# headupinclouds/cvsteer

Hardware: AMD Instinct MI355X
Metric: Mpix/s for G2+H2 7-basis filter+steer at 4096x4096 f32; % HBM roofline (higher is better)
Workload: dtype f32

## Files before the change

cvsteer_amd/csrc/cvs_api.cpp:

```cpp
#include <hip/hip_runtime_api.h>

#include <algorithm>
#include <atomic>
#include <chrono>
#include <condition_variable>
#include <cmath>
#include <cstdio>
#include <cstdlib>
#include <cstring>
#include <limits>
#include <map>
#include <mutex>
#include <set>
#include <tuple>
#include <new>
#include <string>
#include <thread>
#include <vector>

#include "cvs_context.h"

using namespace cvs;

namespace {
// ... 191 lines not shown
    for (int o = 0; o < 5; ++o)
        if ((rc = out_ref(c, outs[o], a.out[o]))) return rc;
    PointOp op = h->kind == CVS_KIND_G2 ? (map ? OP_G2_STEER_MAP : OP_G2_STEER_SCALAR)
                                        : (map ? OP_G4_STEER_MAP : OP_G4_STEER_SCALAR);
    a.nt_stores = use_nt_stores(h, (size_t)a.rows * a.cols);
    a.nt_loads = a.nt_stores;
    HIP_TRY(h, launch_point(op, a, h->stream));
    return finish(c);
}

int g4_pipe_stage(cvs_handle h, const cvs_plane* const outs[8], int nframes, size_t out_fstride)
{
    Call c;
    int rc = begin(h, c, {outs[0], outs[1], outs[2], outs[3], outs[4], outs[5], outs[6], outs[7]});
    if (rc) return rc;
    G4PipeArgs a{};
    a.rows = h->rows;
    a.cols = h->cols;
    a.frames = nframes;
    a.atan_mode = h->atan_mode;
    a.find_on_e = h->find_on;
    for (int p = 0; p < h->nb; ++p) {
        const PlaneRef r = state_ref(h, p);
        a.in[p] = {r.p, r.pitch, h->frame_stride};
    }
    if (h->persist) {
        for (int i = 0; i < 5; ++i) {
            const PlaneRef r = state_ref(h, h->nb + i);
            a.out[G4P_C1 + i] = {r.p, r.pitch, h->frame_stride};
        }
    }
    for (int k = 0; k < 8; ++k) {
        PlaneRef r;
        if ((rc = out_ref(c, outs[k], r))) return rc;
        a.out[G4P_G + k] = {r.p, r.pitch, out_fstride};
    }
    a.nt_stores = use_nt_stores(h, (size_t)a.rows * a.cols * nframes);
    a.nt_loads = a.nt_stores;
    HIP_TRY(h, launch_g4_pipeline(a, h->stream));
    h->have_basis = h->have_orient = h->persist != 0;
    return finish(c);
}

int g4_pipeline_one(cvs_handle h, const cvs_plane* image, const cvs_plane* const outs[8], int nframes, int frame)
{
    const int rc = do_setup(h, image, CVS_SETUP_BASIS, false, 0.f, nullptr, nullptr, nullptr, nframes, frame);
    return rc ? rc : g4_pipe_stage(h, outs, 1, 0);
}

int g4_pipeline_frames(cvs_handle h, const cvs_plane* images, int n, const cvs_plane* outs, bool all_dev)
{
    auto frame_outs = [&](int i, const cvs_plane* po[8]) {
        for (int k = 0; k < 8; ++k) po[k] = (outs && outs[(size_t)i * 8 + k].data) ? &outs[(size_t)i * 8 + k] : nullptr;
    };
    bool block = all_dev;
    ptrdiff_t d_out = 0;
    bool have_stride = false;
    for (int i = 1; i < n && block; ++i)
        for (int k = 0; k < 8 && block && outs; ++k) {
            const cvs_plane &o0 = outs[k], &oi = outs[(size_t)i * 8 + k];
            if ((o0.data == nullptr) != (oi.data == nullptr)) block = false;
            else if (o0.data) {
                const ptrdiff_t dk = oi.data - o0.data;
                if (!have_stride) { d_out = dk / i; have_stride = true; }
                block = dk == d_out * i && d_out > 0 && oi.step == o0.step;
            }
        }
    int rc;
    if (!block) {
        for (int i = 0; i < n; ++i) {
            const cvs_plane* po[8];
            frame_outs(i, po);
            if ((rc = g4_pipeline_one(h, &images[i], po, n, i))) return rc;
        }
        h->cur_frame = 0;
        return CVS_OK;
    }
    for (int i = 0; i < n; ++i)
        if ((rc = do_setup(h, &images[i], CVS_SETUP_BASIS, false, 0.f, nullptr, nullptr, nullptr, n, i))) return rc;
    h->cur_frame = 0;
    const cvs_plane* po[8];
    frame_outs(0, po);
    return g4_pipe_stage(h, po, n, (size_t)d_out);
}

}

extern "C" {

int cvs_abi_version(void) { return CVS_ABI_VERSION; }

const char* cvs_status_string(int s)
{
    switch (s) {
        case CVS_OK: return "ok";
        case CVS_E_BADARG: return "bad argument";
        case CVS_E_SIZE: return "bad size";
        case CVS_E_HIP: return "HIP error";
        case CVS_E_NOMEM: return "out of memory";
        case CVS_E_STATE: return "state not available";
        case CVS_E_UNSUPPORTED: return "unsupported for this kind";
    }
    return "unknown status";
}

int cvs_num_basis(int kind) { return host_num_basis(kind); }

int cvs_make_taps(int kind, int idx, int width, float spacing, float* out)
{
    return host_make_taps(kind, idx, width, spacing, out) ? CVS_E_BADARG : CVS_OK;
}

int cvs_basis_taps(int kind, int p, int* kx, int* ky) { return host_basis_taps(kind, p, kx, ky) ? CVS_E_BADARG : CVS_OK; }

int cvs_steer_weights(int kind, float theta, float* out) { return host_steer_weights(kind, theta, out) ? CVS_E_BADARG : CVS_OK; }

int cvs_create(int kind, int width, float spacing, int device, cvs_handle* out)
{
    if (!out) return CVS_E_BADARG;
    *out = nullptr;
    const int nb = host_num_basis(kind);
    if (nb == 0 || width < 1 || width > kMaxWidth) return CVS_E_BADARG;
    int ndev = 0;
    if (hipGetDeviceCount(&ndev) != hipSuccess || ndev <= 0) return CVS_E_HIP;
    if (device < 0 || device >= ndev) return CVS_E_BADARG;
    if (hipSetDevice(device) != hipSuccess) return CVS_E_HIP;
    cvs_context* h = new (std::nothrow) cvs_context();
    if (!h) return CVS_E_NOMEM;
    h->kind = kind;
    h->width = width;
    h->spacing = spacing;
    h->nb = nb;
    h->device = device;
    std::memset(h->taps, 0, sizeof(h->taps));
    for (int i = 0; i < nb; ++i) host_make_taps(kind, i, width, spacing, h->taps[i]);
    const EnvOpts eo = env_opts();
    if (eo.autotune >= 0) h->autotune = eo.autotune;
    if (eo.layout >= 0) h->layout = eo.layout;
    if (eo.pyr_strip >= 0) h->pyr_strip = eo.pyr_strip;
    *out = h;
    return CVS_OK;
}

int cvs_destroy(cvs_handle h)
{
    if (!h) return CVS_E_BADARG;
    (void)hipSetDevice(h->device);
    release_state(h);
    if (h->arena || h->frame_tab || h->point_out) (void)hipStreamSynchronize(h->stream);
    if (h->arena) (void)hipFree(h->arena);
    if (h->frame_tab) (void)hipFree(h->frame_tab);
    if (h->point_out) (void)hipFree(h->point_out);
    if (h->ev_order) (void)hipEventDestroy(h->ev_order);
    for (hipEvent_t e : h->band_ev) (void)hipEventDestroy(e);
    if (h->s_up) (void)hipStreamDestroy(h->s_up);
    if (h->s_down) (void)hipStreamDestroy(h->s_down);
    delete h;
    return CVS_OK;
}

int cvs_release_cached_memory(void)
{
    pool_release_all();
    return CVS_OK;
}

const char* cvs_last_error(cvs_handle h) { return h ? h->err.c_str() : "null handle"; }

int cvs_set_stream(cvs_handle h, void* s)
{
    if (!h) return CVS_E_BADARG;
    hipStream_t ns = static_cast<hipStream_t>(s);
    if (ns == h->stream) return CVS_OK;
    hipStreamCaptureStatus c0 = hipStreamCaptureStatusNone, c1 = hipStreamCaptureStatusNone;
    (void)hipStreamIsCapturing(h->stream, &c0);
    (void)hipStreamIsCapturing(ns, &c1);
    (void)hipGetLastError();
    if (h->used && c0 == hipStreamCaptureStatusNone && c1 == hipStreamCaptureStatusNone) {
        HIP_TRY(h, hipSetDevice(h->device));
        if (!h->ev_order) HIP_TRY(h, hipEventCreateWithFlags(&h->ev_order, hipEventDisableTiming));
        HIP_TRY(h, hipEventRecord(h->ev_order, h->stream));
        HIP_TRY(h, hipStreamWaitEvent(ns, h->ev_order, 0));
    }
    h->stream = ns;
    return CVS_OK;
}

int cvs_set_option(cvs_handle h, int option, int value)
{
    if (!h) return CVS_E_BADARG;
    switch (option) {
        case CVS_OPT_ATAN_MODE:
            if (value != 0 && value != 1) return fail(h, CVS_E_BADARG, "atan mode");
            h->atan_mode = value;
            return CVS_OK;
        case CVS_OPT_STRIP_ROWS:
            if (value < 0 || value > 1 << 20) return fail(h, CVS_E_BADARG, "strip rows");
            h->strip_rows = value;
            return CVS_OK;
        case CVS_OPT_FIND_ON:
            if (value != 0 && value != 1) return fail(h, CVS_E_BADARG, "find_on");
            h->find_on = value;
            return CVS_OK;
        case CVS_OPT_G4_EXTENSIONS:
            if (value != 0 && value != 1) return fail(h, CVS_E_BADARG, "g4 extensions");
            h->g4_ext = value;
            return CVS_OK;
        case CVS_OPT_PERSIST_STATE:
            if (value != 0 && value != 1) return fail(h, CVS_E_BADARG, "persist");
            h->persist = value;
            return CVS_OK;
        case CVS_OPT_AUTOTUNE:
            if (value != 0 && value != 1) return fail(h, CVS_E_BADARG, "autotune");
            h->autotune = value;
            return CVS_OK;
        case CVS_OPT_BLOCK_ORDER:
            if (value != -1 && value != 0 && value != kOrderXcdColumns && value != kOrderDynamic) return fail(h, CVS_E_BADARG, "block order");
            h->block_order = value;
            return CVS_OK;
        case CVS_OPT_HOST_OVERLAP:
            if (value != 0 && value != 1) return fail(h, CVS_E_BADARG, "host overlap");
            h->host_overlap = value;
            return CVS_OK;
        case CVS_OPT_STATE_LAYOUT:
            if (value < 0 || value > 3) return fail(h, CVS_E_BADARG, "state layout");
            h->layout = value;
            return CVS_OK;
    }
    return fail(h, CVS_E_BADARG, "unknown option");
}

int cvs_get_option(cvs_handle h, int option, int* value)
{
    if (!h || !value) return CVS_E_BADARG;
    switch (option) {
        case CVS_OPT_ATAN_MODE: *value = h->atan_mode; return CVS_OK;
        case CVS_OPT_STRIP_ROWS: *value = h->strip_rows; return CVS_OK;
        case CVS_OPT_FIND_ON: *value = h->find_on; return CVS_OK;
        case CVS_OPT_BLOCK_ORDER: *value = h->block_order; return CVS_OK;
        case CVS_OPT_HOST_OVERLAP: *value = h->host_overlap; return CVS_OK;
        case CVS_OPT_AUTOTUNE: *value = h->autotune; return CVS_OK;
        case CVS_OPT_PERSIST_STATE: *value = h->persist; return CVS_OK;
        case CVS_OPT_G4_EXTENSIONS: *value = h->g4_ext; return CVS_OK;
        case CVS_OPT_STATE_LAYOUT: *value = h->layout; return CVS_OK;
    }
    return fail(h, CVS_E_BADARG, "unknown option");
}

int cvs_get_launch_info(cvs_handle h, cvs_launch_info* out)
{
    if (!h || !out) return CVS_E_BADARG;
    const uint32_t n = out->struct_size;
    if (n < sizeof(uint32_t)) return fail(h, CVS_E_BADARG, "cvs_launch_info.struct_size not set");
    cvs_launch_info li = h->last;
    li.struct_size = (uint32_t)std::min<size_t>(n, sizeof(li));
    std::memcpy(out, &li, li.struct_size);
    return CVS_OK;
}

int cvs_taps(cvs_handle h, int idx, float* out)
{
    if (!h || !out || idx < 0 || idx >= h->nb) return CVS_E_BADARG;
    std::memcpy(out, h->taps[idx], (2 * h->width + 1) * sizeof(float));
    return CVS_OK;
}

int cvs_kind(cvs_handle h, int* kind, int* width, float* spacing)
{
    if (!h) return CVS_E_BADARG;
    if (kind) *kind = h->kind;
    if (width) *width = h->width;
    if (spacing) *spacing = h->spacing;
    return CVS_OK;
}

int cvs_shape(cvs_handle h, int* rows, int* cols)
{
    if (!h) return CVS_E_BADARG;
    if (rows) *rows = h->have_basis ? h->rows : 0;
    if (cols) *cols = h->have_basis ? h->cols : 0;
    return CVS_OK;
}

int cvs_sync(cvs_handle h)
{
    if (!h) return CVS_E_BADARG;
    HIP_TRY(h, hipSetDevice(h->device));
    HIP_TRY(h, hipStreamSynchronize(h->stream));
    return CVS_OK;
}

int cvs_setup(cvs_handle h, const cvs_plane* image, unsigned flags)
{
    return do_setup(h, image, flags, false, 0.f, nullptr, nullptr);
}

int cvs_setup_steer(cvs_handle h, const cvs_plane* image, unsigned flags, float theta, const cvs_plane* g, const cvs_plane* hq)
{
    return do_setup(h, image, flags, true, theta, g, hq);
}

int cvs_setup_pyr(cvs_handle h, const cvs_plane* image, unsigned flags, const cvs_plane* next_level)
{
    if (!h) return CVS_E_BADARG;
    if (!next_level) return fail(h, CVS_E_BADARG, "next_level");
    return do_setup(h, image, flags, false, 0.f, nullptr, nullptr, nullptr, 1, 0, 0, 0, next_level);
// ... 520 lines not shown
```

cvsteer_amd/csrc/cvs_batch.cpp:

```cpp
#include <dlfcn.h>
#include <hip/hip_runtime_api.h>
#include <rccl/rccl.h>

#include <algorithm>
#include <cstdio>
#include <cstdlib>
#include <cstring>
#include <condition_variable>
#include <mutex>
#include <new>
#include <string>
#include <thread>
#include <vector>

#include "cvsteer_hip.h"

namespace {

struct Rccl {
    void* so = nullptr;
    ncclResult_t (*GetUniqueId)(ncclUniqueId*) = nullptr;
    ncclResult_t (*CommInitRank)(ncclComm_t*, int, ncclUniqueId, int) = nullptr;
    ncclResult_t (*CommInitAll)(ncclComm_t*, int, const int*) = nullptr;
    ncclResult_t (*CommDestroy)(ncclComm_t) = nullptr;
    ncclResult_t (*GroupStart)() = nullptr;
    ncclResult_t (*GroupEnd)() = nullptr;
    ncclResult_t (*Send)(const void*, size_t, ncclDataType_t, int, ncclComm_t, hipStream_t) = nullptr;
    ncclResult_t (*Recv)(void*, size_t, ncclDataType_t, int, ncclComm_t, hipStream_t) = nullptr;
    ncclResult_t (*Broadcast)(const void*, void*, size_t, ncclDataType_t, int, ncclComm_t, hipStream_t) = nullptr;
    ncclResult_t (*AllReduce)(const void*, void*, size_t, ncclDataType_t, ncclRedOp_t, ncclComm_t, hipStream_t) = nullptr;
    const char* (*GetErrorString)(ncclResult_t) = nullptr;
    std::string why;
};

Rccl* rccl(std::string* why = nullptr)
{
    static Rccl r;
    static std::once_flag once;
    std::call_once(once, [] {
        const char* env = std::getenv("CVS_RCCL_LIB");
        const char* names[] = {env, "librccl.so.1", "librccl.so", "/opt/rocm/lib/librccl.so.1", "/opt/rocm/lib/librccl.so"};
        for (const char* n : names) {
            if (!n || !*n) continue;
            r.so = dlopen(n, RTLD_NOW | RTLD_GLOBAL);
            if (r.so) break;
        }
        if (!r.so) {
            r.why = std::string("cannot load librccl: ") + (dlerror() ? dlerror() : "not found");
            return;
        }
        bool ok = true;
        auto sym = [&](const char* name) {
            void* p = dlsym(r.so, name);
            if (!p) { ok = false; r.why = std::string("librccl lacks ") + name; }
            return p;
        };
        r.GetUniqueId = reinterpret_cast<decltype(r.GetUniqueId)>(sym("ncclGetUniqueId"));
        r.CommInitRank = reinterpret_cast<decltype(r.CommInitRank)>(sym("ncclCommInitRank"));
        r.CommInitAll = reinterpret_cast<decltype(r.CommInitAll)>(sym("ncclCommInitAll"));
        r.CommDestroy = reinterpret_cast<decltype(r.CommDestroy)>(sym("ncclCommDestroy"));
        r.GroupStart = reinterpret_cast<decltype(r.GroupStart)>(sym("ncclGroupStart"));
        r.GroupEnd = reinterpret_cast<decltype(r.GroupEnd)>(sym("ncclGroupEnd"));
        r.Send = reinterpret_cast<decltype(r.Send)>(sym("ncclSend"));
        r.Recv = reinterpret_cast<decltype(r.Recv)>(sym("ncclRecv"));
        r.Broadcast = reinterpret_cast<decltype(r.Broadcast)>(sym("ncclBroadcast"));
        r.AllReduce = reinterpret_cast<decltype(r.AllReduce)>(sym("ncclAllReduce"));
        r.GetErrorString = reinterpret_cast<decltype(r.GetErrorString)>(sym("ncclGetErrorString"));
        if (!ok) {
            dlclose(r.so);
            r.so = nullptr;
        }
    });
    if (!r.so && why) *why = r.why;
    return r.so ? &r : nullptr;
}

void shard_range(int n, int world, int rank, int* lo, int* hi)
{
    *lo = (int)(((long long)rank * n + world - 1) / world);
    *hi = (int)(((long long)(rank + 1) * n + world - 1) / world);
}

enum { TRANSPORT_NONE = 0, TRANSPORT_RCCL = 1, TRANSPORT_COPY = 2 };

struct DevBuf {
    float* p = nullptr;
    size_t elems = 0;
};

struct Slot {
    int rank = 0, device = 0;
    hipStream_t stream = nullptr;
    cvs_handle h = nullptr;
    std::vector<cvs_handle> level;
    std::vector<DevBuf> level_img;
    ncclComm_t comm = nullptr;
    DevBuf in, out, image;
    DevBuf out8;
    int last_n = 0, last_k = 0, last_rows = 0, last_cols = 0;
    bool last_staged = false;
    hipEvent_t ev[4] = {nullptr, nullptr, nullptr, nullptr};
    hipStream_t up = nullptr, down = nullptr;
    std::vector<hipEvent_t> host_ev;
    int* agree = nullptr;
};

}

struct cvs_batch_context {
    int kind = 0, width = 0, world = 0, transport = TRANSPORT_NONE;
    int g4_ext = 0;
    float spacing = 0.f;
    float u8_gain = 0.f;
    std::vector<Slot> slots;
    int pyr_levels = 0, pyr_root = 0;
    std::string err;
};

namespace {

int fail(cvs_batch b, int code, const std::string& what)
{
    if (b) b->err = what;
    return code;
}

#define B_HIP(b, expr)                                                                                   \
    do {                                                                                                 \
        hipError_t e__ = (expr);                                                                         \
        if (e__ != hipSuccess) return fail(b, e__ == hipErrorOutOfMemory ? CVS_E_NOMEM : CVS_E_HIP,      \
                                           std::string(#expr) + ": " + hipGetErrorString(e__));         \
    } while (0)

#define B_NCCL(b, expr)                                                                                  \
    do {                                                                                                 \
        ncclResult_t r__ = (expr);                                                                       \
        if (r__ != ncclSuccess) return fail(b, CVS_E_HIP, std::string(#expr) + ": " + rccl()->GetErrorString(r__)); \
    } while (0)

#define B_CVS(b, h, expr)                                                                                \
    do {                                                                                                 \
        int rc__ = (expr);                                                                               \
        if (rc__ != CVS_OK) return fail(b, rc__, std::string(#expr) + ": " + cvs_last_error(h));         \
    } while (0)

int reserve(cvs_batch b, Slot& s, DevBuf& buf, size_t elems)
{
    if (elems <= buf.elems) return CVS_OK;
    B_HIP(b, hipSetDevice(s.device));
    if (buf.p) {
        B_HIP(b, hipStreamSynchronize(s.stream));
        B_HIP(b, hipFree(buf.p));
        buf = DevBuf();
    }
    B_HIP(b, hipMalloc(&buf.p, elems * sizeof(float)));
    buf.elems = elems;
    return CVS_OK;
}

Slot* local(cvs_batch b, int rank)
{
    for (Slot& s : b->slots)
        if (s.rank == rank) return &s;
    return nullptr;
}

int init_slot(cvs_batch b, Slot& s)
// ... 75 lines not shown
        return g.end(b);
    }
    for (const Move& m : moves) {
        Slot* s = local(b, m.src_rank);
        Slot* d = local(b, m.dst_rank);
        if (!s || !d) return fail(b, CVS_E_UNSUPPORTED, "copy transport needs both ranks in this process");
        B_HIP(b, hipSetDevice(s->device));
        hipEvent_t e;
        B_HIP(b, hipEventCreateWithFlags(&e, hipEventDisableTiming));
        B_HIP(b, hipEventRecord(e, s->stream));
        B_HIP(b, hipSetDevice(d->device));
        B_HIP(b, hipStreamWaitEvent(d->stream, e, 0));
        B_HIP(b, hipMemcpyAsync(m.dst, m.src, m.count * sizeof(float), hipMemcpyDeviceToDevice, d->stream));
        hipEvent_t done;
        B_HIP(b, hipEventCreateWithFlags(&done, hipEventDisableTiming));
        B_HIP(b, hipEventRecord(done, d->stream));
        B_HIP(b, hipSetDevice(s->device));
        B_HIP(b, hipStreamWaitEvent(s->stream, done, 0));
        B_HIP(b, hipEventDestroy(e));
        B_HIP(b, hipEventDestroy(done));
    }
    return CVS_OK;
}

int agree(cvs_batch b, int local_rc, uint32_t geometry_hash)
{
    static const bool force = std::getenv("CVS_BATCH_FORCE_AGREE") != nullptr;
    if (b->transport != TRANSPORT_RCCL || ((int)b->slots.size() == b->world && !force)) return local_rc;
    Rccl* R = rccl();
    const int h31 = (int)(geometry_hash & 0x3fffffffu);
    int mine[4] = {local_rc, h31, -h31, 0};
    int rc = CVS_OK;
    std::string err;
    for (Slot& s : b->slots) {
        if (hipSetDevice(s.device) != hipSuccess || hipMemcpyAsync(s.agree, mine, sizeof(mine), hipMemcpyHostToDevice, s.stream) != hipSuccess) {
            (void)hipGetLastError();
            rc = CVS_E_HIP;
            err = "status agreement: the status could not be staged on the device";
        }
    }
    {
        GroupGuard g(R);
        g.start();
        for (Slot& s : b->slots) {
            if (!g.ok()) break;
            g.hip(hipSetDevice(s.device), "hipSetDevice");
            if (g.ok()) g.nccl(R->AllReduce(s.agree, s.agree, 4, ncclInt32, ncclMin, s.comm, s.stream), "ncclAllReduce");
        }
        const int grc = g.end(b);
        if (grc != CVS_OK) return grc;
    }
    if (rc != CVS_OK) return fail(b, rc, err);
    int agreed[4] = {0, 0, 0, 0};
    for (Slot& s : b->slots) {
        B_HIP(b, hipSetDevice(s.device));
        B_HIP(b, hipMemcpyAsync(agreed, s.agree, sizeof(agreed), hipMemcpyDeviceToHost, s.stream));
        B_HIP(b, hipStreamSynchronize(s.stream));
        if (agreed[0] != CVS_OK && local_rc == CVS_OK)
            return fail(b, agreed[0], "a peer rank cannot run this call (status " + std::to_string(agreed[0]) + "); nothing was queued");
        if (agreed[1] != -agreed[2] && local_rc == CVS_OK)
            return fail(b, CVS_E_BADARG, "the ranks were called with different geometries / options; nothing was queued");
    }
    return local_rc;
}

uint32_t hash_ints(std::initializer_list<long long> v)
{
    uint64_t h = 1469598103934665603ull;
    for (long long x : v) {
        h ^= (uint64_t)x;
        h *= 1099511628211ull;
    }
    return (uint32_t)(h ^ (h >> 32));
}

int record_all(cvs_batch b, int which)
{
    for (Slot& s : b->slots) {
        B_HIP(b, hipSetDevice(s.device));
        B_HIP(b, hipEventRecord(s.ev[which], s.stream));
    }
    return CVS_OK;
}

int sync_all(cvs_batch b)
{
    for (Slot& s : b->slots) {
        B_HIP(b, hipSetDevice(s.device));
        B_HIP(b, hipStreamSynchronize(s.stream));
    }
    return CVS_OK;
}

void fill_timing(cvs_batch b, cvs_batch_timing* t)
{
    if (!t) return;
    t->scatter_ms = t->compute_ms = t->gather_ms = 0.0;
    for (Slot& s : b->slots) {
        float ms[3] = {0.f, 0.f, 0.f};
        (void)hipSetDevice(s.device);
        for (int i = 0; i < 3; ++i) (void)hipEventElapsedTime(&ms[i], s.ev[i], s.ev[i + 1]);
        t->scatter_ms = std::max(t->scatter_ms, (double)ms[0]);
        t->compute_ms = std::max(t->compute_ms, (double)ms[1]);
        t->gather_ms = std::max(t->gather_ms, (double)ms[2]);
    }
}

bool dense_device(const cvs_plane* p, int rows, int cols)
{
    return p && p->data && p->mem == CVS_MEM_DEVICE && p->rows == rows && p->cols == cols && p->step == (size_t)cols * sizeof(float);
}

bool host_plane(const cvs_plane* p, int rows, int cols, bool u8 = false)
{
    return p && p->data && p->mem == (u8 ? (CVS_MEM_HOST | CVS_DEPTH_U8) : CVS_MEM_HOST) && p->rows == rows && p->cols == cols &&
           p->step >= (size_t)cols * (u8 ? 1 : sizeof(float));
}

struct HostRun {
    cvs_batch b;
    const cvs_batch_cfg* cfg;
    const cvs_plane *inputs, *outputs;
    int sel[8], K;
    bool u8;
    bool out8;
};

int host_rank(const HostRun& R, Slot& s, std::string& err, double ms[3])
{
    cvs_batch b = R.b;
    const int rows = R.cfg->rows, cols = R.cfg->cols, K = R.K;
    const size_t plane = (size_t)rows * cols, rowb = (size_t)cols * sizeof(float);
    int lo, hi;
    shard_range(R.cfg->n_frames, b->world, s.rank, &lo, &hi);
    const int n = hi - lo;
    ms[0] = ms[1] = ms[2] = 0.0;
    if (!n) {
        s.last_n = 0;
        s.last_staged = true;
        return CVS_OK;
    }
#define H_TRY(expr)                                                                              \
    do {                                                                                         \
        hipError_t e__ = (expr);                                                                 \
        if (e__ != hipSuccess) { err = std::string(#expr) + ": " + hipGetErrorString(e__); return e__ == hipErrorOutOfMemory ? CVS_E_NOMEM : CVS_E_HIP; } \
    } while (0)
    H_TRY(hipSetDevice(s.device));
    if (!s.up) {
        H_TRY(hipStreamCreateWithFlags(&s.up, hipStreamNonBlocking));
        H_TRY(hipStreamCreateWithFlags(&s.down, hipStreamNonBlocking));
    }
    int persist = 1;
    (void)cvs_get_option(s.h, CVS_OPT_PERSIST_STATE, &persist);
    std::vector<int> c0(1, 0);
    if (persist) c0.push_back(n);
    else
        for (int sz = std::max(1, n / 32); c0.back() < n; sz *= 2) c0.push_back((n - c0.back() <= sz + sz / 2 || c0.size() >= 5) ? n : c0.back() + sz);
    const int nchunks = (int)c0.size() - 1;
    while ((int)s.host_ev.size() < 4 + 2 * nchunks) {
        hipEvent_t ev = nullptr;
        H_TRY(s.host_ev.size() < 4 ? hipEventCreate(&ev) : hipEventCreateWithFlags(&ev, hipEventDisableTiming));
        s.host_ev.push_back(ev);
    }
    hipEvent_t* t = s.host_ev.data();
    hipEvent_t* up_ev = s.host_ev.data() + 4;
    hipEvent_t* done_ev = s.host_ev.data() + 4 + nchunks;
    std::mutex mu;
    std::condition_variable cv;
    int queued = 0;
    bool stop = false;
    int drc = CVS_OK;
    std::string derr;
    std::thread down;
    if (R.cfg->gather) {
        down = std::thread([&]() {
            if (hipSetDevice(s.device) != hipSuccess) { drc = CVS_E_HIP; derr = "hipSetDevice"; return; }
            for (int c = 0; c < nchunks; ++c) {
                {
                    std::unique_lock<std::mutex> lk(mu);
                    cv.wait(lk, [&] { return queued > c || stop; });
                    if (stop) return;
                }
                hipError_t e = hipStreamWaitEvent(s.down, done_ev[c], 0);
                if (c == 0 && e == hipSuccess) e = hipEventRecord(t[2], s.down);
                if (R.out8) {
                    const uint8_t* dev8 = reinterpret_cast<const uint8_t*>(s.out8.p);
                    size_t first = (size_t)c0[c] * K, count = 0;
                    uint8_t* run_dst = nullptr;
                    auto flush = [&]() {
                        if (count && e == hipSuccess) e = hipMemcpyAsync(run_dst, dev8 + first * plane, count * plane, hipMemcpyDeviceToHost, s.down);
                        count = 0;
                    };
                    for (int i = c0[c]; e == hipSuccess && i < c0[c + 1]; ++i)
                        for (int j = 0; e == hipSuccess && j < K; ++j) {
                            const cvs_plane& o = R.outputs[(size_t)(lo + i) * 8 + R.sel[j]];
                            uint8_t* dst = reinterpret_cast<uint8_t*>(o.data);
                            const size_t idx = (size_t)i * K + j;
                            if (o.step != (size_t)cols) {
                                flush();
                                if (e == hipSuccess) e = hipMemcpy2DAsync(dst, o.step, dev8 + idx * plane, (size_t)cols, (size_t)cols, rows, hipMemcpyDeviceToHost, s.down);
                                continue;
                            }
                            if (count && dst == run_dst + count * plane) { ++count; continue; }
                            flush();
                            first = idx; run_dst = dst; count = 1;
                        }
                    flush();
                } else {
                    size_t first = (size_t)c0[c] * K, count = 0;
                    float* run_dst = nullptr;
                    auto flush = [&]() {
                        if (count && e == hipSuccess) e = hipMemcpyAsync(run_dst, s.out.p + first * plane, count * plane * sizeof(float), hipMemcpyDeviceToHost, s.down);
                        count = 0;
                    };
                    for (int i = c0[c]; e == hipSuccess && i < c0[c + 1]; ++i)
                        for (int j = 0; e == hipSuccess && j < K; ++j) {
                            const cvs_plane& o = R.outputs[(size_t)(lo + i) * 8 + R.sel[j]];
                            const size_t idx = (size_t)i * K + j;
                            if (o.step != rowb) {
                                flush();
                                if (e == hipSuccess) e = hipMemcpy2DAsync(o.data, o.step, s.out.p + idx * plane, rowb, rowb, rows, hipMemcpyDeviceToHost, s.down);
                                continue;
                            }
                            if (count && o.data == run_dst + count * plane) { ++count; continue; }
                            flush();
                            first = idx; run_dst = o.data; count = 1;
                        }
                    flush();
                }
                if (e != hipSuccess) { drc = CVS_E_HIP; derr = std::string("download: ") + hipGetErrorString(e); return; }
            }
            hipError_t e = hipEventRecord(t[3], s.down);
            if (e == hipSuccess) e = hipStreamSynchronize(s.down);
            if (e != hipSuccess) { drc = CVS_E_HIP; derr = std::string("download: ") + hipGetErrorString(e); }
        });
    }
    auto stop_down = [&](bool failed) {
        if (down.joinable()) {
            {
                std::lock_guard<std::mutex> lk(mu);
                if (failed) stop = true;
            }
            cv.notify_all();
            down.join();
        }
    };
    int rc = CVS_OK;
    hipError_t e = hipEventRecord(t[0], s.up);
    for (int c = 0; c < nchunks && e == hipSuccess && rc == CVS_OK; ++c) {
        {
            const size_t esz = R.u8 ? 1 : sizeof(float), frame_b = plane * esz;
            uint8_t* dev = reinterpret_cast<uint8_t*>(s.in.p);
            int first = c0[c], count = 0;
            const uint8_t* run_src = nullptr;
            auto flush = [&]() {
                if (count && e == hipSuccess) e = hipMemcpyAsync(dev + (size_t)first * frame_b, run_src, (size_t)count * frame_b, hipMemcpyHostToDevice, s.up);
                count = 0;
            };
            for (int i = c0[c]; e == hipSuccess && i < c0[c + 1]; ++i) {
                const cvs_plane& im = R.inputs[lo + i];
                const uint8_t* src = reinterpret_cast<const uint8_t*>(im.data);
                if (im.step != (size_t)cols * esz) {
                    flush();
                    if (e == hipSuccess) e = hipMemcpy2DAsync(dev + (size_t)i * frame_b, (size_t)cols * esz, im.data, im.step, (size_t)cols * esz, rows, hipMemcpyHostToDevice, s.up);
                    continue;
                }
                if (count && src == run_src + (size_t)count * frame_b) { ++count; continue; }
                flush();
                first = i; run_src = src; count = 1;
            }
            flush();
        }
        if (e == hipSuccess) e = hipEventRecord(up_ev[c], s.up);
        if (e == hipSuccess && c == nchunks - 1) e = hipEventRecord(t[1], s.up);
        if (e == hipSuccess) e = hipStreamWaitEvent(s.stream, up_ev[c], 0);
        if (e != hipSuccess) break;
        const int cn = c0[c + 1] - c0[c];
        std::vector<cvs_plane> im(cn), ou((size_t)cn * 8);
        std::memset(ou.data(), 0, ou.size() * sizeof(cvs_plane));
        for (int i = 0; i < cn; ++i) {
            if (R.u8) im[i] = cvs_plane{reinterpret_cast<float*>(reinterpret_cast<uint8_t*>(s.in.p) + (size_t)(c0[c] + i) * plane), rows, cols, (size_t)cols, CVS_MEM_DEVICE | CVS_DEPTH_U8};
            else im[i] = cvs_plane{s.in.p + (size_t)(c0[c] + i) * plane, rows, cols, rowb, CVS_MEM_DEVICE};
            for (int j = 0; j < K; ++j)
                ou[(size_t)i * 8 + R.sel[j]] = cvs_plane{s.out.p + ((size_t)(c0[c] + i) * K + j) * plane, rows, cols, rowb, CVS_MEM_DEVICE};
        }
        rc = cvs_pipeline_batch(s.h, im.data(), cn, ou.data());
        if (rc != CVS_OK) { err = std::string("cvs_pipeline_batch: ") + cvs_last_error(s.h); break; }
        if (R.out8) {
            const size_t m = (size_t)cn * K;
            std::vector<cvs_plane> src(m);
            std::vector<uint8_t*> dst(m);
            for (size_t q = 0; q < m; ++q) {
                src[q] = cvs_plane{s.out.p + ((size_t)c0[c] * K + q) * plane, rows, cols, rowb, CVS_MEM_DEVICE};
                dst[q] = reinterpret_cast<uint8_t*>(s.out8.p) + ((size_t)c0[c] * K + q) * plane;
            }
            rc = b->u8_gain > 0.f ? cvs_convert_u8_batch(s.h, src.data(), (int)m, b->u8_gain, 0.f, dst.data(), (size_t)cols, CVS_MEM_DEVICE)
                                  : cvs_normalize_u8_batch(s.h, src.data(), (int)m, dst.data(), (size_t)cols, CVS_MEM_DEVICE);
            if (rc != CVS_OK) { err = std::string("cvs_*_u8_batch: ") + cvs_last_error(s.h); break; }
        }
        e = hipEventRecord(done_ev[c], s.stream);
        if (e == hipSuccess) {
            {
                std::lock_guard<std::mutex> lk(mu);
                queued = c + 1;
            }
            cv.notify_all();
        }
    }
    const bool failed = e != hipSuccess || rc != CVS_OK;
    if (e != hipSuccess) { err = std::string("upload: ") + hipGetErrorString(e); rc = CVS_E_HIP; }
// ... 480 lines not shown
```

cvsteer_amd/csrc/cvs_context.h:

```cpp
#pragma once
#include <hip/hip_runtime_api.h>

#include <initializer_list>
#include <string>
#include <vector>

#include "cvs_internal.h"
#include "cvsteer_hip.h"

struct cvs_context {
    static constexpr int kMaxBasis = cvs::kMaxBasis, kMaxTaps = cvs::kMaxTaps;
    using StateBlock = cvs::StateBlock;
    using BatchFrame = cvs::BatchFrame;
    int kind = 0, width = 0, nb = 0, device = 0;
    float spacing = 0.f;
    hipStream_t stream = nullptr;
    float taps[kMaxBasis][kMaxTaps];
    int rows = 0, cols = 0;
    struct PlaneGroup {
        int first = 0, count = 0;
        size_t off = 0;
        size_t pitch = 0;
        size_t stride = 0;
    };
    PlaneGroup grp[3];
    int ngrp = 0;
    size_t dense_pitch = 0;
    size_t layout_stride = 0;
    float* state = nullptr;
    size_t state_elems = 0;
    StateBlock sb;
    bool have_basis = false, have_orient = false;
    int num_frames = 1, cur_frame = 0;
    size_t frame_stride = 0;
    BatchFrame* frame_tab = nullptr;
    int frame_tab_cap = 0;
    float* arena = nullptr;
    size_t arena_elems = 0, arena_used = 0;
    float* point_out = nullptr;
    const void* last_image = nullptr;
    int layout = 1;
    int atan_mode = 0, strip_rows = 0, find_on = 0, block_order = -1, persist = 1, g4_ext = 0, autotune = 1;
    cvs_launch_info last{};
    int pyr_strip = 1;
    hipEvent_t ev_order = nullptr;
    hipStream_t s_up = nullptr, s_down = nullptr;
    std::vector<hipEvent_t> band_ev;
    int host_overlap = 1;
    bool used = false;
    std::string err;
};

static inline hipError_t copy_rows(void* dst, size_t dpitch, const void* src, size_t spitch, size_t width, size_t rows,
                                   hipMemcpyKind kind, hipStream_t stream)
{
    if (dpitch == width && spitch == width) return hipMemcpyAsync(dst, src, width * rows, kind, stream);
    return hipMemcpy2DAsync(dst, dpitch, src, spitch, width, rows, kind, stream);
}

namespace cvs {

int fail(cvs_handle h, int code, const char* what);
int fail_hip(cvs_handle h, hipError_t e, const char* where);

#define HIP_TRY(h, expr)                                        \
    do {                                                        \
        hipError_t e__ = (expr);                                \
        if (e__ != hipSuccess) return fail_hip(h, e__, #expr);  \
    } while (0)

struct RelaxedCapture {
    hipStreamCaptureMode mode = hipStreamCaptureModeRelaxed;
    RelaxedCapture() { (void)hipThreadExchangeStreamCaptureMode(&mode); }
    ~RelaxedCapture() { (void)hipThreadExchangeStreamCaptureMode(&mode); }
    RelaxedCapture(const RelaxedCapture&) = delete;
    RelaxedCapture& operator=(const RelaxedCapture&) = delete;
};

inline size_t round_up(size_t v, size_t m) { return (v + m - 1) / m * m; }
inline bool is_u8(const cvs_plane* p) { return (p->mem & CVS_DEPTH_U8) != 0; }
inline int mem_of(const cvs_plane* p) { return p->mem & 0xff; }

struct Pending {
    const cvs_plane* host;
    float* dev;
    size_t pitch;
};

struct Call {
    cvs_handle h;
    std::vector<Pending> outs;
    bool touched_host = false;
    size_t need = 0;
    bool defer = false;
    const cvs_plane* deferred_image = nullptr;
    uint8_t* deferred_u8 = nullptr;
    size_t deferred_u8_pitch = 0;
    bool u8_direct = false;
};

int check_plane(cvs_handle h, const cvs_plane* p, const char* name, bool allow_u8 = false);
bool planes_overlap(const cvs_plane* a, const cvs_plane* b);
int check_no_overlap(cvs_handle h, const cvs_plane* input, const cvs_plane* const* outs, int n);
int check_point_overlaps(cvs_handle h, std::initializer_list<const cvs_plane*> ins, std::initializer_list<const cvs_plane*> outs);
int check_same(cvs_handle h, const cvs_plane* p, int rows, int cols);
int arena_reserve(cvs_handle h, size_t elems);
float* arena_take(cvs_handle h, size_t elems);
size_t u8_stage_elems(const cvs_plane* p);
size_t staged_elems(const cvs_plane* p);
int in_ref(Call& c, const cvs_plane* p, PlaneRef& r);
int out_ref(Call& c, const cvs_plane* p, PlaneRef& r);
int finish(Call& c);
int begin(cvs_handle h, Call& c, std::initializer_list<const cvs_plane*> planes, size_t extra = 0);
float* state_plane(cvs_handle h, int idx);
PlaneRef state_ref(cvs_handle h, int idx);
const cvs_context::PlaneGroup& state_group(cvs_handle h, int idx);
void fill_state_args(cvs_handle h, BasisArgs& a, bool orient);
void pool_give(StateBlock& blk);
void pool_release_all();
void release_state(cvs_handle h);
bool state_interleaved(cvs_handle h, int rows, size_t dense_pitch);
int ensure_state(cvs_handle h, int rows, int cols, int nframes = 1);
bool state_merge_fits(cvs_handle h, int rows, size_t dense_pitch);
void layout_state(cvs_handle h, bool merge_orient);

int default_strip_rows(cvs_handle h, int rows, int cols, bool fresh_input = false);
int use_nt_stores(cvs_handle h, size_t npix);
struct EnvOpts {
    int autotune = -1, layout = -1, pyr_strip = -1, batch_ways = -1, nt_stores = -1, warm = -1, wgcap = -1, lit = -1, verbose = 0;
    long pool_mb = 4096;
};
EnvOpts env_opts();
struct TuneToken {
    void* entry = nullptr;
    int cand = 0, calls = 1;
    double npix = 0;
    hipEvent_t e0 = nullptr, e1 = nullptr;
};
int tune_begin(cvs_handle h, BasisArgs& a, int variant, bool fresh_input, TuneToken& tok);
void tune_end(cvs_handle h, const TuneToken& tok);
void note_launch(cvs_handle h, const BasisArgs& a);

int host_pipeline(cvs_handle h, Call& c, BasisArgs& a, float* scr);

}
```

cvsteer_amd/csrc/cvs_handle.cpp:

```cpp
#include <hip/hip_runtime_api.h>

#include <algorithm>
#include <atomic>
#include <chrono>
#include <condition_variable>
#include <cmath>
#include <cstdio>
#include <cstdlib>
#include <cstring>
#include <limits>
#include <map>
#include <mutex>
#include <set>
#include <tuple>
#include <new>
#include <string>
#include <thread>
#include <vector>

#include "cvs_context.h"

namespace cvs {

EnvOpts env_opts()
{
    static std::mutex mu;
    static std::string cached_text;
    static EnvOpts cached;
    static bool have = false;
    const char* e = std::getenv("CVS_OPTS");
    const std::string text = e ? e : "";
    std::lock_guard<std::mutex> lock(mu);
    if (have && text == cached_text) return cached;
    EnvOpts v;
    size_t pos = 0;
    while (pos < text.size()) {
        size_t end = text.find(',', pos);
        if (end == std::string::npos) end = text.size();
        const std::string item = text.substr(pos, end - pos);
        pos = end + 1;
        const size_t eq = item.find('=');
        if (eq == std::string::npos) continue;
        const std::string name = item.substr(0, eq);
        const long val = std::atol(item.c_str() + eq + 1);
        if (name == "autotune") v.autotune = val != 0;
        else if (name == "layout") v.layout = (int)std::max(0L, std::min(3L, val));
        else if (name == "pyr_strip") v.pyr_strip = val != 0;
        else if (name == "batch_ways") v.batch_ways = (int)std::max(1L, val);
        else if (name == "nt_stores") v.nt_stores = val != 0;
        else if (name == "warm") v.warm = (int)std::max(0L, std::min(16L, val));
        else if (name == "wgcap") v.wgcap = (int)std::max(0L, std::min(8L, val));
        else if (name == "lit") v.lit = val != 0;
        else if (name == "verbose") v.verbose = val != 0;
        else if (name == "pool_mb") v.pool_mb = val;
        else std::fprintf(stderr, "[cvsteer] CVS_OPTS: unknown name '%s' ignored\n", name.c_str());
    }
    cached = v;
    cached_text = text;
    have = true;
    return v;
}

int fail(cvs_handle h, int code, const char* what)
{
    if (h) h->err = what;
    return code;
}

int fail_hip(cvs_handle h, hipError_t e, const char* where)
{
    if (h) h->err = std::string(where) + ": " + hipGetErrorString(e);
    return e == hipErrorOutOfMemory ? CVS_E_NOMEM : CVS_E_HIP;
}



int check_plane(cvs_handle h, const cvs_plane* p, const char* name, bool allow_u8)
{
    if (!p) return fail(h, CVS_E_BADARG, name);
    if (p->rows <= 0 || p->cols <= 0) return fail(h, CVS_E_SIZE, "empty plane");
    if (!p->data) return fail(h, CVS_E_BADARG, name);
    if ((p->mem & ~(0xff | CVS_DEPTH_U8)) || (is_u8(p) && !allow_u8)) return fail(h, CVS_E_BADARG, "bad mem / depth flags");
    if (mem_of(p) != CVS_MEM_HOST && mem_of(p) != CVS_MEM_DEVICE) return fail(h, CVS_E_BADARG, "bad mem kind");
    if (is_u8(p)) {
        if (p->step < (size_t)p->cols) return fail(h, CVS_E_SIZE, "bad step");
    } else if (p->step < (size_t)p->cols * sizeof(float) || p->step % sizeof(float)) {
        return fail(h, CVS_E_SIZE, "bad step");
    } else if (reinterpret_cast<uintptr_t>(p->data) % alignof(float)) {
        return fail(h, CVS_E_BADARG, "f32 plane not aligned to 4 bytes");
    }
    return CVS_OK;
}

bool planes_overlap(const cvs_plane* a, const cvs_plane* b)
{
    if (!a || !b || !a->data || !b->data || mem_of(a) != mem_of(b)) return false;
    auto width = [](const cvs_plane* p) { return (size_t)p->cols * (is_u8(p) ? 1 : sizeof(float)); };
    auto extent = [&](const cvs_plane* p) { return (size_t)(p->rows - 1) * p->step + width(p); };
    const uintptr_t pa = reinterpret_cast<uintptr_t>(a->data), pb = reinterpret_cast<uintptr_t>(b->data);
    if (pa + extent(a) <= pb || pb + extent(b) <= pa) return false;
    if (a->step != b->step || a->step == 0) return true;
    const cvs_plane* lo = pa <= pb ? a : b;
    const cvs_plane* hi = pa <= pb ? b : a;
    const size_t d = (size_t)(reinterpret_cast<uintptr_t>(hi->data) - reinterpret_cast<uintptr_t>(lo->data));
    const size_t r = d / lo->step, c = d % lo->step;
    return (r < (size_t)lo->rows && c < width(lo)) || (r + 1 < (size_t)lo->rows && c + width(hi) > lo->step);
}

int check_no_overlap(cvs_handle h, const cvs_plane* input, const cvs_plane* const* outs, int n)
{
    for (int i = 0; i < n; ++i) {
        if (!outs[i] || !outs[i]->data) continue;
        if (input && planes_overlap(outs[i], input)) return fail(h, CVS_E_BADARG, "an output plane overlaps the input image");
        for (int j = i + 1; j < n; ++j)
            if (outs[j] && planes_overlap(outs[i], outs[j])) return fail(h, CVS_E_BADARG, "two output planes overlap each other");
    }
    return CVS_OK;
}

int check_point_overlaps(cvs_handle h, std::initializer_list<const cvs_plane*> ins, std::initializer_list<const cvs_plane*> outs)
{
    for (auto o = outs.begin(); o != outs.end(); ++o) {
        if (!*o || !(*o)->data) continue;
        for (const cvs_plane* i : ins)
            if (i && planes_overlap(*o, i) && !((*o)->data == i->data && (*o)->step == i->step))
                return fail(h, CVS_E_BADARG, "an output plane overlaps an input plane without being it");
        for (auto q = o + 1; q != outs.end(); ++q)
            if (*q && planes_overlap(*o, *q)) return fail(h, CVS_E_BADARG, "two output planes overlap each other");
    }
    return CVS_OK;
}

int check_same(cvs_handle h, const cvs_plane* p, int rows, int cols)
{
    if (p->rows != rows || p->cols != cols) return fail(h, CVS_E_SIZE, "plane size mismatch");
    return CVS_OK;
}


int arena_reserve(cvs_handle h, size_t elems)
{
    if (elems <= h->arena_elems) return CVS_OK;
    if (h->arena) {
        HIP_TRY(h, hipStreamSynchronize(h->stream));
        HIP_TRY(h, hipFree(h->arena));
        h->arena = nullptr;
        h->arena_elems = 0;
    }
    HIP_TRY(h, hipMalloc(&h->arena, elems * sizeof(float)));
    h->arena_elems = elems;
    return CVS_OK;
}

float* arena_take(cvs_handle h, size_t elems)
{
    float* p = h->arena + h->arena_used;
    h->arena_used += round_up(elems, 64);
    return p;
}

size_t u8_stage_elems(const cvs_plane* p) { return round_up(round_up((size_t)p->cols, 256) * p->rows / 4 + 64, 64); }

size_t staged_elems(const cvs_plane* p)
{
    if (!p) return 0;
    const size_t plane = round_up(round_up((size_t)p->cols, 64) * p->rows, 64);
    if (is_u8(p))
        return plane + (mem_of(p) == CVS_MEM_HOST ? u8_stage_elems(p) : 0);
    return mem_of(p) == CVS_MEM_HOST ? plane : 0;
}

int in_ref(Call& c, const cvs_plane* p, PlaneRef& r)
{
    cvs_handle h = c.h;
    if (is_u8(p) && c.u8_direct) {
        if (mem_of(p) == CVS_MEM_DEVICE) {
            r = {p->data, p->step};
            return CVS_OK;
        }
        const size_t bpitch = round_up((size_t)p->cols, 256);
        uint8_t* b = reinterpret_cast<uint8_t*>(arena_take(h, u8_stage_elems(p)));
        HIP_TRY(h, copy_rows(b, bpitch, p->data, p->step, (size_t)p->cols, p->rows, hipMemcpyHostToDevice, h->stream));
        c.touched_host = true;
        r = {reinterpret_cast<float*>(b), bpitch};
        return CVS_OK;
    }
    if (is_u8(p)) {
        const size_t pitch = round_up((size_t)p->cols, 64);
        float* d = arena_take(h, pitch * p->rows);
        const uint8_t* src = reinterpret_cast<const uint8_t*>(p->data);
        size_t sstep = p->step;
        if (mem_of(p) == CVS_MEM_HOST) {
            const size_t bpitch = round_up((size_t)p->cols, 256);
            uint8_t* b = reinterpret_cast<uint8_t*>(arena_take(h, round_up(bpitch * p->rows / 4 + 64, 64)));
            if (c.defer) {
                c.deferred_image = p;
                c.deferred_u8 = b;
                c.deferred_u8_pitch = bpitch;
                r = {d, pitch};
                return CVS_OK;
            }
            HIP_TRY(h, copy_rows(b, bpitch, p->data, p->step, (size_t)p->cols, p->rows, hipMemcpyHostToDevice, h->stream));
            c.touched_host = true;
            src = b;
            sstep = bpitch;
        }
        HIP_TRY(h, launch_u8_to_f32(src, sstep, p->rows, p->cols, d, pitch, h->stream));
// ... 267 lines not shown
```

cvsteer_amd/csrc/cvs_host.cpp:

```cpp
#include <hip/hip_runtime_api.h>

#include <algorithm>
#include <atomic>
#include <chrono>
#include <condition_variable>
#include <cmath>
#include <cstdio>
#include <cstdlib>
#include <cstring>
#include <limits>
#include <map>
#include <mutex>
#include <set>
#include <tuple>
#include <new>
#include <string>
#include <thread>
#include <vector>

#include "cvs_context.h"

namespace cvs {

int host_pipeline(cvs_handle h, Call& c, BasisArgs& a, float* scr)
{
    const int W = h->width;
    int nbands = 8;
    int per = (a.rows + nbands - 1) / nbands;
    per = std::max(a.strip_rows, (per + a.strip_rows - 1) / a.strip_rows * a.strip_rows);
    nbands = (a.rows + per - 1) / per;
    if (!h->s_up) {
        HIP_TRY(h, hipStreamCreateWithFlags(&h->s_up, hipStreamNonBlocking));
        HIP_TRY(h, hipStreamCreateWithFlags(&h->s_down, hipStreamNonBlocking));
    }
    while ((int)h->band_ev.size() < 2 * nbands + 1) {
        hipEvent_t e;
        HIP_TRY(h, hipEventCreateWithFlags(&e, hipEventDisableTiming));
        h->band_ev.push_back(e);
    }
    hipEvent_t* up = h->band_ev.data();
    hipEvent_t* comp = h->band_ev.data() + nbands;
    hipEvent_t start = h->band_ev[2 * nbands];
    HIP_TRY(h, hipEventRecord(start, h->stream));
    HIP_TRY(h, hipStreamWaitEvent(h->s_up, start, 0));
    HIP_TRY(h, hipStreamWaitEvent(h->s_down, start, 0));
    a.block_order = 0;
    note_launch(h, a);

    std::mutex mu;
    std::condition_variable cv;
    int enqueued = 0;
    bool abort_dl = false;
    hipError_t dl_err = hipSuccess;
    const std::vector<Pending> outs = c.outs;
    const int rows = a.rows, device = h->device;
    hipStream_t s_down = h->s_down;
    std::thread downloader;
    if (!outs.empty()) {
        downloader = std::thread([&, rows, device, s_down, per, nbands] {
            hipError_t e = hipSetDevice(device);
            for (int b = 0; b < nbands && e == hipSuccess; ++b) {
                {
                    std::unique_lock<std::mutex> lock(mu);
                    cv.wait(lock, [&] { return enqueued > b || abort_dl; });
                    if (abort_dl) break;
                }
                const int lo = b * per, hi = std::min(rows, lo + per);
                e = hipStreamWaitEvent(s_down, comp[b], 0);
                for (const Pending& o : outs) {
                    if (e != hipSuccess) break;
                    if (o.host->step == o.pitch * sizeof(float) && o.host->step == (size_t)o.host->cols * sizeof(float)) {
                        e = hipMemcpyAsync(reinterpret_cast<char*>(o.host->data) + (size_t)lo * o.host->step, o.dev + (size_t)lo * o.pitch,
                                           (size_t)(hi - lo) * o.host->step, hipMemcpyDeviceToHost, s_down);
                        continue;
                    }
                    e = copy_rows(reinterpret_cast<char*>(o.host->data) + (size_t)lo * o.host->step, o.host->step, o.dev + (size_t)lo * o.pitch,
                                         o.pitch * sizeof(float), (size_t)o.host->cols * sizeof(float), hi - lo, hipMemcpyDeviceToHost, s_down);
                }
            }
            if (e == hipSuccess) e = hipStreamSynchronize(s_down);
            dl_err = e;
        });
    }
    auto stop = [&](int rc) {
        {
            std::lock_guard<std::mutex> lock(mu);
            abort_dl = true;
        }
        cv.notify_all();
        if (downloader.joinable()) downloader.join();
        return rc;
    };
    const cvs_plane* img = c.deferred_image;
    int up_to = 0;
    for (int b = 0; b < nbands; ++b) {
        const int lo = b * per, hi = std::min(a.rows, lo + per);
        if (img) {
            const int need = std::min(a.rows, hi + W);
            if (need > up_to) {
                hipError_t e;
                if (c.deferred_u8) {
                    e = copy_rows(c.deferred_u8 + (size_t)up_to * c.deferred_u8_pitch, c.deferred_u8_pitch,
                                         reinterpret_cast<const char*>(img->data) + (size_t)up_to * img->step, img->step, (size_t)img->cols, need - up_to,
                                         hipMemcpyHostToDevice, h->s_up);
                    if (e == hipSuccess)
                        e = launch_u8_to_f32(c.deferred_u8 + (size_t)up_to * c.deferred_u8_pitch, c.deferred_u8_pitch, need - up_to, img->cols,
                                             const_cast<float*>(a.in) + (size_t)up_to * a.in_pitch, a.in_pitch, h->s_up);
                } else {
                    e = copy_rows(const_cast<float*>(a.in) + (size_t)up_to * a.in_pitch, a.in_pitch * sizeof(float),
                                         reinterpret_cast<const char*>(img->data) + (size_t)up_to * img->step, img->step, (size_t)img->cols * sizeof(float),
                                         need - up_to, hipMemcpyHostToDevice, h->s_up);
                }
                if (e != hipSuccess) return stop(fail_hip(h, e, "host pipeline upload"));
                up_to = need;
            }
            hipError_t e = hipEventRecord(up[b], h->s_up);
            if (e == hipSuccess) e = hipStreamWaitEvent(h->stream, up[b], 0);
            if (e != hipSuccess) return stop(fail_hip(h, e, "host pipeline ordering"));
        }
        BasisArgs ab = a;
        ab.out_row_lo = lo;
        ab.out_row_hi = hi;
        hipError_t e = launch_basis(h->kind, h->width, h->taps, ab, scr, h->stream);
        if (e == hipSuccess) e = hipEventRecord(comp[b], h->stream);
        if (e != hipSuccess) return stop(fail_hip(h, e, "host pipeline launch"));
        {
            std::lock_guard<std::mutex> lock(mu);
            enqueued = b + 1;
        }
        cv.notify_all();
    }
    if (downloader.joinable()) downloader.join();
    if (dl_err != hipSuccess) return fail_hip(h, dl_err, "host pipeline download");
    HIP_TRY(h, hipStreamSynchronize(h->stream));
    c.outs.clear();
    return CVS_OK;
}

}
```

Before: 165,300.

## Reuse a persistent download worker thread and use geometric host pipeline bands

Replaces the per-call download thread in the host pipeline with a persistent worker stored on the handle, driven by a mutex and condition variable, so repeated calls skip thread creation and teardown. Band edges now come from a shared planner that uses geometrically growing bands (small first band) unless an env option asks for equal bands, which lets the first download begin sooner. The contiguous fast-path memcpy branch is dropped in favour of copy_rows, which already handles that case. The cost is extra lifecycle complexity: the worker must be stopped in destroy, and it holds a pointer to the caller's event array.

```diff
diff --git a/cvsteer_amd/csrc/cvs_api.cpp b/cvsteer_amd/csrc/cvs_api.cpp
--- a/cvsteer_amd/csrc/cvs_api.cpp
+++ b/cvsteer_amd/csrc/cvs_api.cpp
@@ -367,6 +367,7 @@
     if (h->frame_tab) (void)hipFree(h->frame_tab);
     if (h->point_out) (void)hipFree(h->point_out);
     if (h->ev_order) (void)hipEventDestroy(h->ev_order);
+    stop_host_worker(h);
     for (hipEvent_t e : h->band_ev) (void)hipEventDestroy(e);
     if (h->s_up) (void)hipStreamDestroy(h->s_up);
     if (h->s_down) (void)hipStreamDestroy(h->s_down);
diff --git a/cvsteer_amd/csrc/cvs_bands.h b/cvsteer_amd/csrc/cvs_bands.h
--- /dev/null
+++ b/cvsteer_amd/csrc/cvs_bands.h
@@ -0,0 +1,23 @@
+#pragma once
+#include <algorithm>
+#include <vector>
+
+namespace cvs {
+
+inline std::vector<int> plan_bands(int total, int quantum, int equal = 0)
+{
+    std::vector<int> e(1, 0);
+    if (total <= 0) return e;
+    quantum = std::max(1, quantum);
+    auto up = [quantum](long v) { return (int)((v + quantum - 1) / quantum * quantum); };
+    if (equal > 0) {
+        const int per = std::max(quantum, up((total + (long)equal - 1) / equal));
+        while (e.back() < total) e.push_back(std::min(total, e.back() + per));
+        return e;
+    }
+    for (long sz = std::max(quantum, up(total / 32)); e.back() < total; sz *= 2)
+        e.push_back((total - e.back() <= sz + sz / 2 || e.size() >= 5) ? total : (int)(e.back() + sz));
+    return e;
+}
+
+}
diff --git a/cvsteer_amd/csrc/cvs_batch.cpp b/cvsteer_amd/csrc/cvs_batch.cpp
--- a/cvsteer_amd/csrc/cvs_batch.cpp
+++ b/cvsteer_amd/csrc/cvs_batch.cpp
@@ -13,6 +13,7 @@
 #include <thread>
 #include <vector>
 
+#include "cvs_bands.h"
 #include "cvsteer_hip.h"
 
 namespace {
@@ -394,10 +395,7 @@
     }
     int persist = 1;
     (void)cvs_get_option(s.h, CVS_OPT_PERSIST_STATE, &persist);
-    std::vector<int> c0(1, 0);
-    if (persist) c0.push_back(n);
-    else
-        for (int sz = std::max(1, n / 32); c0.back() < n; sz *= 2) c0.push_back((n - c0.back() <= sz + sz / 2 || c0.size() >= 5) ? n : c0.back() + sz);
+    const std::vector<int> c0 = persist ? std::vector<int>{0, n} : cvs::plan_bands(n, 1);
     const int nchunks = (int)c0.size() - 1;
     while ((int)s.host_ev.size() < 4 + 2 * nchunks) {
         hipEvent_t ev = nullptr;
diff --git a/cvsteer_amd/csrc/cvs_context.h b/cvsteer_amd/csrc/cvs_context.h
--- a/cvsteer_amd/csrc/cvs_context.h
+++ b/cvsteer_amd/csrc/cvs_context.h
@@ -7,6 +7,10 @@
 
 #include "cvs_internal.h"
 #include "cvsteer_hip.h"
+
+namespace cvs {
+struct HostWorker;
+}
 
 struct cvs_context {
     static constexpr int kMaxBasis = cvs::kMaxBasis, kMaxTaps = cvs::kMaxTaps;
@@ -46,6 +50,7 @@
     hipEvent_t ev_order = nullptr;
     hipStream_t s_up = nullptr, s_down = nullptr;
     std::vector<hipEvent_t> band_ev;
+    cvs::HostWorker* dl = nullptr;
     int host_overlap = 1;
     bool used = false;
     std::string err;
@@ -128,6 +133,7 @@
 int use_nt_stores(cvs_handle h, size_t npix);
 struct EnvOpts {
     int autotune = -1, layout = -1, pyr_strip = -1, batch_ways = -1, nt_stores = -1, warm = -1, wgcap = -1, lit = -1, verbose = 0;
+    int host_bands = 0;
     long pool_mb = 4096;
 };
 EnvOpts env_opts();
@@ -142,5 +148,6 @@
 void note_launch(cvs_handle h, const BasisArgs& a);
 
 int host_pipeline(cvs_handle h, Call& c, BasisArgs& a, float* scr);
+void stop_host_worker(cvs_handle h);
 
 }
diff --git a/cvsteer_amd/csrc/cvs_handle.cpp b/cvsteer_amd/csrc/cvs_handle.cpp
--- a/cvsteer_amd/csrc/cvs_handle.cpp
+++ b/cvsteer_amd/csrc/cvs_handle.cpp
@@ -53,6 +53,7 @@
         else if (name == "lit") v.lit = val != 0;
         else if (name == "verbose") v.verbose = val != 0;
         else if (name == "pool_mb") v.pool_mb = val;
+        else if (name == "host_bands") v.host_bands = (int)std::max(0L, std::min(64L, val));
         else std::fprintf(stderr, "[cvsteer] CVS_OPTS: unknown name '%s' ignored\n", name.c_str());
     }
     cached = v;
diff --git a/cvsteer_amd/csrc/cvs_host.cpp b/cvsteer_amd/csrc/cvs_host.cpp
--- a/cvsteer_amd/csrc/cvs_host.cpp
+++ b/cvsteer_amd/csrc/cvs_host.cpp
@@ -18,17 +18,76 @@
 #include <thread>
 #include <vector>
 
+#include "cvs_bands.h"
 #include "cvs_context.h"
 
 namespace cvs {
 
+
+struct HostWorker {
+    std::mutex mu;
+    std::condition_variable cv;
+    std::thread th;
+    std::vector<Pending> outs;
+    std::vector<int> edges;
+    const hipEvent_t* comp = nullptr;
+    int posted = 0;
+    bool open = false, done = false, abort = false, quit = false;
+    hipError_t err = hipSuccess;
+};
+
+static void download_loop(HostWorker* w, int device, hipStream_t s_down)
+{
+    const hipError_t dev_err = hipSetDevice(device);
+    std::unique_lock<std::mutex> lock(w->mu);
+    for (;;) {
+        w->cv.wait(lock, [w] { return w->quit || (w->open && !w->done); });
+        if (w->quit) return;
+        hipError_t e = dev_err;
+        const int nbands = (int)w->edges.size() - 1;
+        for (int b = 0; b < nbands && e == hipSuccess; ++b) {
+            w->cv.wait(lock, [w, b] { return w->posted > b || w->abort; });
+            if (w->abort) break;
+            lock.unlock();
+            const int lo = w->edges[b], hi = w->edges[b + 1];
+            e = hipStreamWaitEvent(s_down, w->comp[b], 0);
+            for (const Pending& o : w->outs) {
+                if (e != hipSuccess) break;
+                e = copy_rows(reinterpret_cast<char*>(o.host->data) + (size_t)lo * o.host->step, o.host->step, o.dev + (size_t)lo * o.pitch,
+                              o.pitch * sizeof(float), (size_t)o.host->cols * sizeof(float), hi - lo, hipMemcpyDeviceToHost, s_down);
+            }
+            lock.lock();
+        }
+        if (e == hipSuccess) {
+            lock.unlock();
+            e = hipStreamSynchronize(s_down);
+            lock.lock();
+        }
+        w->err = e;
+        w->done = true;
+        w->cv.notify_all();
+    }
+}
+
+void stop_host_worker(cvs_handle h)
+{
+    HostWorker* w = h->dl;
+    if (!w) return;
+    {
+        std::lock_guard<std::mutex> lock(w->mu);
+        w->quit = true;
+    }
+    w->cv.notify_all();
+    if (w->th.joinable()) w->th.join();
+    delete w;
+    h->dl = nullptr;
+}
+
 int host_pipeline(cvs_handle h, Call& c, BasisArgs& a, float* scr)
 {
     const int W = h->width;
-    int nbands = 8;
-    int per = (a.rows + nbands - 1) / nbands;
-    per = std::max(a.strip_rows, (per + a.strip_rows - 1) / a.strip_rows * a.strip_rows);
-    nbands = (a.rows + per - 1) / per;
+    const std::vector<int> edges = plan_bands(a.rows, a.strip_rows, env_opts().host_bands);
+    const int nbands = (int)edges.size() - 1;
     if (!h->s_up) {
         HIP_TRY(h, hipStreamCreateWithFlags(&h->s_up, hipStreamNonBlocking));
         HIP_TRY(h, hipStreamCreateWithFlags(&h->s_down, hipStreamNonBlocking));
@@ -47,54 +106,51 @@
     a.block_order = 0;
     note_launch(h, a);
 
-    std::mutex mu;
-    std::condition_variable cv;
-    int enqueued = 0;
-    bool abort_dl = false;
-    hipError_t dl_err = hipSuccess;
-    const std::vector<Pending> outs = c.outs;
-    const int rows = a.rows, device = h->device;
-    hipStream_t s_down = h->s_down;
-    std::thread downloader;
-    if (!outs.empty()) {
-        downloader = std::thread([&, rows, device, s_down, per, nbands] {
-            hipError_t e = hipSetDevice(device);
-            for (int b = 0; b < nbands && e == hipSuccess; ++b) {
-                {
-                    std::unique_lock<std::mutex> lock(mu);
-                    cv.wait(lock, [&] { return enqueued > b || abort_dl; });
-                    if (abort_dl) break;
-                }
-                const int lo = b * per, hi = std::min(rows, lo + per);
-                e = hipStreamWaitEvent(s_down, comp[b], 0);
-                for (const Pending& o : outs) {
-                    if (e != hipSuccess) break;
-                    if (o.host->step == o.pitch * sizeof(float) && o.host->step == (size_t)o.host->cols * sizeof(float)) {
-                        e = hipMemcpyAsync(reinterpret_cast<char*>(o.host->data) + (size_t)lo * o.host->step, o.dev + (size_t)lo * o.pitch,
-                                           (size_t)(hi - lo) * o.host->step, hipMemcpyDeviceToHost, s_down);
-                        continue;
-                    }
-                    e = copy_rows(reinterpret_cast<char*>(o.host->data) + (size_t)lo * o.host->step, o.host->step, o.dev + (size_t)lo * o.pitch,
-                                         o.pitch * sizeof(float), (size_t)o.host->cols * sizeof(float), hi - lo, hipMemcpyDeviceToHost, s_down);
-                }
+    HostWorker* w = nullptr;
+    if (!c.outs.empty()) {
+        if (!h->dl) {
+            HostWorker* nw = new (std::nothrow) HostWorker;
+            if (!nw) return fail(h, CVS_E_NOMEM, "host pipeline: download worker");
+            try {
+                nw->th = std::thread(download_loop, nw, h->device, h->s_down);
+            } catch (const std::exception&) {
+                delete nw;
+                return fail(h, CVS_E_NOMEM, "host pipeline: cannot start the download worker");
             }
-            if (e == hipSuccess) e = hipStreamSynchronize(s_down);
-            dl_err = e;
-        });
+            h->dl = nw;
+        }
+        w = h->dl;
+        {
+            std::lock_guard<std::mutex> lock(w->mu);
+            w->outs = c.outs;
+            w->edges = edges;
+            w->comp = comp;
+            w->posted = 0;
+            w->done = w->abort = false;
+            w->err = hipSuccess;
+            w->open = true;
+        }
+        w->cv.notify_all();
     }
+    auto close_job = [w](bool abort) {
+        if (!w) return hipSuccess;
+        std::unique_lock<std::mutex> lock(w->mu);
+        if (abort) {
+            w->abort = true;
+            w->cv.notify_all();
+        }
+        w->cv.wait(lock, [w] { return w->done; });
+        w->open = false;
+        return w->err;
+    };
     auto stop = [&](int rc) {
-        {
-            std::lock_guard<std::mutex> lock(mu);
-            abort_dl = true;
-        }
-        cv.notify_all();
-        if (downloader.joinable()) downloader.join();
+        (void)close_job(true);
         return rc;
     };
     const cvs_plane* img = c.deferred_image;
     int up_to = 0;
     for (int b = 0; b < nbands; ++b) {
-        const int lo = b * per, hi = std::min(a.rows, lo + per);
+        const int lo = edges[b], hi = edges[b + 1];
         if (img) {
             const int need = std::min(a.rows, hi + W);
             if (need > up_to) {
@@ -124,13 +180,15 @@
         hipError_t e = launch_basis(h->kind, h->width, h->taps, ab, scr, h->stream);
         if (e == hipSuccess) e = hipEventRecord(comp[b], h->stream);
         if (e != hipSuccess) return stop(fail_hip(h, e, "host pipeline launch"));
-        {
-            std::lock_guard<std::mutex> lock(mu);
-            enqueued = b + 1;
+        if (w) {
+            {
+                std::lock_guard<std::mutex> lock(w->mu);
+                w->posted = b + 1;
+            }
+            w->cv.notify_all();
         }
-        cv.notify_all();
     }
-    if (downloader.joinable()) downloader.join();
+    const hipError_t dl_err = close_job(false);
     if (dl_err != hipSuccess) return fail_hip(h, dl_err, "host pipeline download");
     HIP_TRY(h, hipStreamSynchronize(h->stream));
     c.outs.clear();
```

New measurement: 165,100, median of 6. Within noise of the previous version (-0.2%).
